# bilkitty/mj_envs

Hardware: AMD Instinct MI355X
Metric: env-steps/sec at N parallel envs, hammer-v0, 1/2/4/8 MI355X (higher is better)
Workload: dtype f32

## Files before the change

include/adroit_wave.h:

```cpp
#ifndef ADROIT_WAVE_H
#define ADROIT_WAVE_H

#include <stddef.h>
#include <stdint.h>

#ifdef __cplusplus
extern "C" {
#endif

typedef struct aw_handle aw_handle;

enum {
  AW_OK = 0,
  AW_EINVAL = -1,
  AW_EBLOB = -2,
  AW_EHIP = -3,
  AW_ENOMEM = -4,
  AW_EUNSUPPORTED = -5
};

enum {
  AW_ST_BADQPOS = 1,
  AW_ST_BADQVEL = 2,
  AW_ST_BADQACC = 4,
// ... 121 lines not shown
                         uint64_t seed, uint64_t draw, float* col, float* light, float* look, void* stream);

int aw_render_entries(const aw_handle* h, int* ngeom, int* nsite);
int aw_render_labels(aw_handle* h, const aw_view* views, int nviews, const float* env_cam,
                     const int32_t* env_ids, int n_sel, const int32_t* lut, int32_t background,
                     int sites, int width, int height, int32_t* labels, float* depth, void* stream);

#define AW_CLOUD_MAXCAND 8192
#define AW_FPS_MAXPOINTS 1024
int aw_render_cloud(aw_handle* h, const aw_view* views, int nviews, const float* env_cam,
                    const int32_t* env_ids, int n_sel, const uint8_t* keep, const float* box,
                    int frame_body, int sites, int width, int height, int cap, float* xyz, int32_t* pix,
                    int32_t* count, void* stream);
int aw_cloud_fps(int n, int cap, const float* xyz, const int32_t* count, int npoints, float* out_xyz,
                 int32_t* out_idx, void* stream);

#define AW_MAX_RAYS 256
typedef struct { float pnt[3], vec[3]; float xmax; int32_t body; uint64_t keep; } aw_ray_rec;
int aw_set_rays(aw_handle* h, const aw_ray_rec* rays, int nrays);
int aw_cast_rays(aw_handle* h, const int32_t* env_ids, int n_sel, const float* env_rays, float* dist,
                 int32_t* entry, void* stream);

int aw_policy_mlp(int n, int in_dim, int hidden, int out_dim, const float* params, const float* obs,
                  float* act, int sample, uint64_t seed, uint64_t step, uint64_t env_offset, void* stream);

#define AW_MAXPAIRCON 8
int aw_collide_test(aw_handle* h, int n, const int32_t* types, const float* pos, const float* mat,
                    const float* size, const float* margin, float* out, int32_t* count, double* out64,
                    void* stream);

int aw_midphase_test(aw_handle* h, int n, const int32_t* pair, const float* pos, const float* quat,
                     const float* size, int32_t* info, float* margin, void* stream);

int aw_stage_profile(unsigned long long* out, int reset);

const char* aw_last_error(void);

#ifdef __cplusplus
}
#endif

#endif
```

mj_envs_amd/_native.py:

```python
from __future__ import annotations

import ctypes
import os
from typing import Optional

import numpy as np

HERE = os.path.dirname(os.path.abspath(__file__))
LIB_PATH = os.environ.get("AW_LIB") or os.path.join(HERE, "libadroit_hip.so")

AW_NDIMS = 21
MAXCON, MAXEFC, MAXDENSE = 48, 192, 128
NCONMAX, NJMAX = 100, 500
ST_BADQPOS, ST_BADQVEL, ST_BADQACC, ST_CON_OVERFLOW, ST_EFC_OVERFLOW, ST_WIDE = 1, 2, 4, 8, 16, 32
ST_OVERFLOW = ST_CON_OVERFLOW | ST_EFC_OVERFLOW


def dump_layout(maxcon=MAXCON, maxefc=MAXEFC):
    c, e = 1768, 1768 + 14 * maxcon
    return dict(xpos=(0, 96), xquat=(96, 128), site_xpos=(224, 96), qacc_smooth=(320, 36),
                qfrc_smooth=(356, 36), qacc=(392, 36), qfrc_constraint=(428, 36), qM=(464, 1296),
                scalars=(1760, 8), con_dist=(c, maxcon), con_pos=(c + maxcon, 3 * maxcon),
                con_frame=(c + 4 * maxcon, 9 * maxcon), con_pair=(c + 13 * maxcon, maxcon),
                efc_force=(e, maxefc), efc_aref=(e + maxefc, maxefc), efc_D=(e + 2 * maxefc, maxefc),
# ... 86 lines not shown
    "aw_random_actions": (_i, [_vp, _u64, _u64, _vp, _vp]),
    "aw_set_env_offset": (_i, [_vp, _u64]),
    "aw_get_state": (_i, [_vp] * 6),
    "aw_set_state": (_i, [_vp] * 7),
    "aw_set_state_ids": (_i, [_vp, _vp, _i, _vp, _i, _vp, _vp, _vp, _vp, _i, _vp, _vp]),
    "aw_get_state_ids": (_i, [_vp, _vp, _i, _vp, _vp, _vp, _vp, _vp]),
    "aw_clone_envs": (_i, [_vp, _vp, _vp, _i, _i, _vp, _vp]),
    "aw_status": (_i, [_vp] * 4),
    "aw_clear_status": (_i, [_vp, _vp]),
    "aw_episode_stats": (_i, [_vp] * 6),
    "aw_episode_totals": (_i, [_vp] * 5),
    "aw_set_episode_totals": (_i, [_vp] * 5),
    "aw_get_episode": (_i, [_vp] * 6),
    "aw_set_episode": (_i, [_vp] * 6),
    "aw_task_eval": (_i, [_vp, _i] + [_vp] * 11),
    "aw_forward_dump": (_i, [_vp, _i, _vp, _vp, _vp]),
    "aw_forward_dump_wide": (_i, [_vp, _i, _vp, _vp, _vp]),
    "aw_dynamics": (_i, [_vp, _vp, _i, _P(DynPoint), _i, _vp, _vp, _vp, _P(DynOut), _vp]),
    "aw_render_depth": (_i, [_vp, _vp, _i, _i, _vp, _vp]),
    "aw_render_rgb": (_i, [_vp, _vp, _vp, _i, _i, _i, _vp, _vp, _vp]),
    "aw_render_views": (_i, [_vp, _P(View), _i, _vp, _vp, _i, _i, _i, _vp, _vp, _vp]),
    "aw_set_appearance": (_i, [_vp, _P(AppearanceBufs), _i]),
    "aw_appearance_defaults": (_i, [_vp, _vp, _vp, _P(_i)]),
    "aw_appearance_sample": (_i, [_vp, _vp, _vp, _vp, _i, _u64, _u64, _vp, _vp, _vp, _vp]),
    "aw_render_entries": (_i, [_vp, _P(_i), _P(_i)]),
    "aw_render_labels": (_i, [_vp, _P(View), _i, _vp, _vp, _i, _vp, _i, _i, _i, _i, _vp, _vp, _vp]),
    "aw_render_cloud": (_i, [_vp, _P(View), _i, _vp, _vp, _i, _vp, _vp] + [_i] * 5 + [_vp] * 4),
    "aw_cloud_fps": (_i, [_i, _i, _vp, _vp, _i, _vp, _vp, _vp]),
    "aw_set_rays": (_i, [_vp, _vp, _i]),
    "aw_cast_rays": (_i, [_vp, _vp, _i, _vp, _vp, _vp, _vp]),
    "aw_policy_mlp": (_i, [_i] * 4 + [_vp, _vp, _vp, _i, _u64, _u64, _u64, _vp]),
    "aw_collide_test": (_i, [_vp, _i] + [_vp] * 9),
    "aw_midphase_test": (_i, [_vp, _i] + [_vp] * 7),
    "aw_stage_profile": (_i, [_vp, _i]),
    "aw_last_error": (ctypes.c_char_p, []),
}
EXPORTS = tuple(ABI)


def data_groups(data) -> int:
    if data is None or data is False:
        return 0
    if data is True:
        return AW_DATA_ALL
    if isinstance(data, int):
        if data & ~AW_DATA_ALL or data < 0:
            raise ValueError(f"data: unknown group bits in {data}")
        return data
    names = (data,) if isinstance(data, str) else tuple(data)
    g = 0
    for k in names:
        if k not in DATA_GROUPS:
            raise ValueError(f"data: unknown group {k!r} (one of {sorted(DATA_GROUPS)})")
        g |= DATA_GROUPS[k]
    return g


class NativeError(RuntimeError):
    pass


def load():
    global _lib
    if _lib is not None:
        return _lib
    if not os.path.exists(LIB_PATH):
# ... 433 lines not shown
        _check(load().aw_render_cloud(self.h, arr, nv, _ptr(env_cam), _ptr(env_ids), n if n_sel is None else int(n_sel),
                                      _host_ptr(kp), _host_ptr(bx), int(frame_body), int(sites), w, h,
                                      0 if cap is None else int(cap), _ptr(xyz), _ptr(pix), _ptr(count), _stream()))

    def collide_test(self, types, pos, mat, size, margin, fp64: bool = False):
        import torch
        n = len(types)
        dev = self.torch_device
        t = lambda a, dt=torch.float32: torch.tensor(np.asarray(a), dtype=dt, device=dev).contiguous()
        out = torch.zeros(n, 8, 7, device=dev)
        cnt = torch.zeros(n, dtype=torch.int32, device=dev)
        out64 = torch.zeros(n, 8, 7, dtype=torch.float64, device=dev) if fp64 else None
        args = [t(types, torch.int32), t(pos), t(mat), t(size), t(margin)]
        _check(load().aw_collide_test(self.h, n, *[_ptr(a) for a in args], _ptr(out), _ptr(cnt), _ptr(out64),
                                      _stream()))
        o = (out64 if fp64 else out).cpu().numpy().astype(np.float64)
        c = cnt.cpu().numpy()
        return [o[i, :c[i]] for i in range(n)]

    def midphase_test(self, pair, pos, quat, size):
        import torch
        n = len(pair)
        dev = self.torch_device
        t = lambda a, dt=torch.float32: torch.tensor(np.asarray(a), dtype=dt, device=dev).contiguous()
        args = [t(pair, torch.int32), t(pos), t(quat), t(size)]
        _require(args[1].numel() == 6 * n and args[2].numel() == 8 * n and args[3].numel() == 6 * n,
                 "midphase_test: pos [n, 2, 3], quat [n, 2, 4], size [n, 2, 3]")
        info = torch.zeros(n, 6, dtype=torch.int32, device=dev)
        mg = torch.zeros(n, device=dev)
        _check(load().aw_midphase_test(self.h, n, *[_ptr(a) for a in args], _ptr(info), _ptr(mg), _stream()))
        i = info.cpu().numpy()
        return dict(keep=i[:, 0], g1=i[:, 1], g2=i[:, 2], cls=i[:, 3], type1=i[:, 4], type2=i[:, 5],
                    margin=mg.cpu().numpy())

    def dynamics(self, out: dict, points=(), env_ids=None, qpos=None, qvel=None, ctrl=None,
                 n_sel: Optional[int] = None, npoints: Optional[int] = None):
        import torch
        pts = list(points)
        arr = (DynPoint * max(len(pts), 1))()
        for k, (kind, idx) in enumerate(pts):
            arr[k].kind, arr[k].id = int(kind), int(idx)
        n, npt = self._n_sel("dynamics", env_ids), len(pts)
        unknown = set(out) - set(DYN_OUTPUTS)
        _require(not unknown, f"dynamics: unknown outputs {sorted(unknown)}")
        c = DynOut()
        for k, t in out.items():
            if _dev(t, f"dynamics: {k}", torch.float32, (n,) + dyn_shape(k, self.nv, self.nbody, npt)) is not None:
                setattr(c, k, t.data_ptr())
        self._rows("dynamics", n, qpos=qpos, qvel=qvel, ctrl=ctrl)
        _check(load().aw_dynamics(self.h, _ptr(env_ids), n if n_sel is None else int(n_sel), arr,
                                  npt if npoints is None else int(npoints), _ptr(qpos), _ptr(qvel), _ptr(ctrl),
                                  ctypes.byref(c), _stream()))

    def set_rays(self, records, nrays: Optional[int] = None):
        rec = None if records is None else np.ascontiguousarray(records, RAY_DTYPE).ravel()
        n = (0 if rec is None else int(rec.size)) if nrays is None else int(nrays)
        _require(rec is None or n <= rec.size or n > AW_MAX_RAYS, "set_rays: nrays exceeds the records given")
        _check(load().aw_set_rays(self.h, None if rec is None or rec.size == 0 else rec.ctypes.data, n))
        self.nrays = n

    def cast_rays(self, dist, entry=None, env_ids=None, env_rays=None, n_sel: Optional[int] = None):
        import torch
        n, R = self._n_sel("cast_rays", env_ids), getattr(self, "nrays", 0)
        _dev(dist, "cast_rays: dist", torch.float32, (n, R))
        _dev(entry, "cast_rays: entry", torch.int32, (n, R))
        _dev(env_rays, "cast_rays: env_rays", torch.float32, (self.n_envs, R, 6))
# ... 28 lines not shown
```

mj_envs_amd/csrc/aw_api.hip:

```cpp
#include <hip/hip_runtime.h>

#include <cmath>
#include <cstddef>
#include <cstdio>
#include <cstdlib>
#include <cstring>
#include <initializer_list>
#include <memory>
#include <string>
#include <vector>

#include "../../include/adroit_wave.h"
#include "../../include/aw_blob.h"
#include "aw_collide.h"
#include "aw_common.h"
#include "aw_handle.h"
#include "aw_model_host.h"
#include "aw_policy.h"
#include "aw_task.h"

using namespace aw;

__global__ void __launch_bounds__(64) k_task_eval(DModel m, int n, const float* qpos, const float* qvel,
                                                  const float* xpos, const float* xquat, const float* sxpos,
                                                  const float* touch, float* obs, float* reward, uint8_t* done,
                                                  uint8_t* goal) {
  __shared__ Env s;
  const int i = blockIdx.x, lane = threadIdx.x;
  if (i >= n) return;
  if (lane < m.nq) { s.qpos[lane] = qpos[(size_t)i * m.nq + lane]; s.qlo[lane] = 0.f; }
  if (lane < m.nv) s.qvel[lane] = qvel[(size_t)i * m.nv + lane];
  for (int k = lane; k < m.nbody * 3; k += 64) (&s.xpos[0][0])[k] = xpos[(size_t)i * m.nbody * 3 + k];
  for (int k = lane; k < m.nbody * 4; k += 64) (&s.xquat[0][0])[k] = xquat[(size_t)i * m.nbody * 4 + k];
  for (int k = lane; k < m.nsite * 3; k += 64) (&s.sxpos[0][0])[k] = sxpos[(size_t)i * m.nsite * 3 + k];
  if (lane == 0) s.touch[0] = touch ? touch[i] : 0.f;
  wsync();
  write_obs(m, s, lane, obs + (size_t)i * m.obs_dim);
  if (lane == 0) {
    float r;
    int dn, gl;
    task_reward(m, s, &r, &dn, &gl);
    reward[i] = r; done[i] = (uint8_t)dn; goal[i] = (uint8_t)gl;
  }
}

AW_DEV void collide_gv(const DModel& m, const GV& a, const GV& b, float margin, Emit& e, int gl) {
  const int lo = a.type, hi = b.type;
  if (hi == GEOM_BOX && lo == GEOM_CAPSULE) {
    c_capsule_box(a, b, margin, e, gl);
    return;
  }
  if (lo != GEOM_PLANE && (lo == GEOM_CYLINDER || hi == GEOM_CYLINDER)) {
// ... 46 lines not shown
  }
  wsync();
  const int nc = s.ncon < MAXPAIRCON ? s.ncon : MAXPAIRCON;
  if (lane == 0) count[i] = nc;
  if (lane < nc) {
    float* o = out + ((size_t)i * MAXPAIRCON + s.con_key[lane]) * 7;
    o[0] = s.con_dist[lane];
    for (int k = 0; k < 3; k++) { o[1 + k] = s.con_pos[lane][k]; o[4 + k] = s.con_nrm[lane][k]; }
  }
}

__global__ void __launch_bounds__(64) k_midphase_test(DModel m, int n, const int* pair, const float* pos,
                                                      const float* quat, const float* size, int* info,
                                                      float* margin) {
  __shared__ Env s;
  const int i = blockIdx.x, lane = threadIdx.x;
  if (i >= n || lane != 0) return;
  const int p = pair[i];
  if ((unsigned)p >= (unsigned)m.npairall) { info[6 * i] = -1; return; }
  const int g[2] = {MD(cp_g1, p), MD(cp_g2, p)};
  for (int q = 0; q < 2; q++) {
    for (int k = 0; k < 3; k++) { s.gxpos[g[q]][k] = pos[6 * i + 3 * q + k]; s.gsize[g[q]][k] = size[6 * i + 3 * q + k]; }
    for (int k = 0; k < 4; k++) s.gxquat[g[q]][k] = quat[8 * i + 4 * q + k];
  }
  const int cls = MD(cp_class, p);
  bool keep = true;
  if (cls == 2) keep = capbox_may_touch(m, s, p);
  else if (cls == 3) keep = boxbox_may_touch(m, s, p);
  else if (cls == 4) keep = mpr_may_touch(m, s, p);
  int* o = info + 6 * i;
  o[0] = keep ? 1 : 0; o[1] = g[0]; o[2] = g[1]; o[3] = cls;
  o[4] = MD(geom_type, g[0]); o[5] = MD(geom_type, g[1]);
  margin[i] = MD(cp_margin, p);
}

__global__ void k_random_actions(int n, int nu, uint64_t seed, uint64_t step, uint64_t env_offset, float* out) {
  int env = blockIdx.x * blockDim.x + threadIdx.x;
  if (env >= n) return;
  const uint32_t genv = (uint32_t)(env_offset + (uint64_t)env);
  for (int blk = 0; blk * 4 < nu; blk++) {
    uint32_t c[4] = {genv, (uint32_t)step, (uint32_t)(step >> 32), (uint32_t)blk};
    philox(c, (uint32_t)seed, (uint32_t)(seed >> 32));
    for (int k = 0; k < 4 && blk * 4 + k < nu; k++) out[(size_t)env * nu + blk * 4 + k] = 2.f * u01(c[k]) - 1.f;
  }
}

AW_DEV float appearance_draw(const float* lo, const float* hi, int i, uint32_t genv, uint64_t seed, uint64_t draw) {
  uint32_t c[4] = {genv, (uint32_t)draw, 0xA99Eu, (uint32_t)(i >> 2)};
  philox(c, (uint32_t)seed, (uint32_t)(seed >> 32));
  return lo[i] + (hi[i] - lo[i]) * u01(c[i & 3]);
}
__global__ void __launch_bounds__(256) k_appearance(int n, int nc, int nl, const float* __restrict__ lo,
                                                    const float* __restrict__ hi, const int* __restrict__ env_ids,
                                                    int row0, uint64_t env_offset, uint64_t seed, uint64_t draw, float* col,
                                                    float* light, float* look) {
  const int i = blockIdx.x * blockDim.x + threadIdx.x, F = nc + nl + AW_LOOK_FLOATS;
  const int row = row0 + (int)blockIdx.y;
  const int env = env_ids ? env_ids[row] : row;
  if (i >= F || (unsigned)env >= (unsigned)n) return;
  const uint32_t genv = (uint32_t)(env_offset + (uint64_t)env);
  float v = appearance_draw(lo, hi, i, genv, seed, draw);
  if (i < nc) {
    if (col) col[(size_t)env * nc + i] = v;
  } else if (i < nc + nl) {
    const int k = (i - nc) % LIGHT_W;
    if (k == 18 || k == 20 || k == 21) v = lo[i];
// ... 840 lines not shown
  const int bs = 256, nb = (n + bs - 1) / bs;
  hipStream_t st = (hipStream_t)stream;
  switch (hidden) {
    case 32: hipLaunchKernelGGL(k_mlp<32>, dim3(nb), dim3(bs), 0, st, n, in_dim, out_dim, params, obs, act, sample, seed, step, env_offset); break;
    case 64: hipLaunchKernelGGL(k_mlp<64>, dim3(nb), dim3(bs), 0, st, n, in_dim, out_dim, params, obs, act, sample, seed, step, env_offset); break;
    default: return fail(AW_EUNSUPPORTED, "aw_policy_mlp: hidden width must be 32 or 64 (two hidden layers)");
  }
  HIPCHK(hipGetLastError());
  return AW_OK;
}

int aw_collide_test(aw_handle* h, int n, const int32_t* types, const float* pos, const float* mat, const float* size,
                    const float* margin, float* out, int32_t* count, double* out64, void* stream) {
  if (!h || n <= 0 || !types || !pos || !mat || !size || !margin || !out || !count)
    return fail(AW_EINVAL, "aw_collide_test: bad arguments");
  HIPCHK(hipSetDevice(h->device));
  hipStream_t st = (hipStream_t)stream;
  hipLaunchKernelGGL(k_collide_test, dim3(n), dim3(64), 0, st, h->m, n, types, pos, mat, size, margin, out, count, out64);
  HIPCHK(hipGetLastError());
  return AW_OK;
}

int aw_midphase_test(aw_handle* h, int n, const int32_t* pair, const float* pos, const float* quat, const float* size,
                     int32_t* info, float* margin, void* stream) {
  if (!h || n <= 0 || !pair || !pos || !quat || !size || !info || !margin)
    return fail(AW_EINVAL, "aw_midphase_test: bad arguments");
  HIPCHK(hipSetDevice(h->device));
  hipStream_t st = (hipStream_t)stream;
  hipLaunchKernelGGL(k_midphase_test, dim3(n), dim3(64), 0, st, h->m, n, pair, pos, quat, size, info, margin);
  HIPCHK(hipGetLastError());
  return AW_OK;
}

int aw_stage_profile(unsigned long long* out, int reset) {
#ifdef AW_STAGE_PROF
  HIPCHK(stage_prof_read(out, reset));
  return AW_OK;
#else
  (void)out; (void)reset;
  return fail(AW_EUNSUPPORTED, "library built without -DAW_STAGE_PROF");
#endif
}

}
```

mj_envs_amd/csrc/aw_common.h:

```cpp
#pragma once
#include <hip/hip_runtime.h>
#include <stdint.h>

#define AW_DEV __device__ __attribute__((always_inline)) inline

namespace aw {

constexpr int MAXV = 36;
constexpr int CHOL_P = 4;
constexpr int VS = 36;
constexpr int MAXB = 32;
constexpr int MAXG = 36;
constexpr int MAXS = 32;
constexpr int MAXT = 44;
constexpr int MAXU = 30;
constexpr int MAXJB = 6;
constexpr int MAXP = 8;
constexpr int MAXLEV = 16;
constexpr int MAXTOUCH = 4;
constexpr int MAXSENS = 72;
constexpr int MAXPAIRCON = 8;
constexpr int NCLASS = 5;

}
// ... 197 lines not shown
                   \
  X(const SensTab*, sens, 1)                                                                      \
            \
  X(const DataTab*, data, 1)

typedef float MRec __attribute__((ext_vector_type(4)));

struct SensTab {
  int n;
  float* out;
  int type[MAXSENS], obj[MAXSENS], adr[MAXSENS];
  int site_type[MAXS];
  float site_size[MAXS * 3];
  int act_dof[MAXU];
};

struct DataTab {
  int groups, max_contacts;
  float *xpos, *xquat, *site_xpos, *qacc, *qfrc_constraint;
  int* counts;
  MRec* contact;
  int geom_id[MAXG];
};

struct MData {
#define AW_X(T, name, n) T name[n];
  AW_MODEL_ARRAYS(AW_X)
#undef AW_X
};

#ifndef AW_MD_AS
#define AW_MD_AS 4
#endif
template <class T>
AW_DEV T mld(const T* base, unsigned i) {
  typedef const __attribute__((address_space(AW_MD_AS))) T GT;
  typedef const __attribute__((address_space(AW_MD_AS))) char GC;
  return *(GT*)((GC*)base + i * (unsigned)sizeof(T));
}
#define MD(name, idx) ::aw::mld(m.d->name, (unsigned)(idx))
template <class T> using gp_t = __attribute__((address_space(1))) T*;
template <class T> AW_DEV gp_t<const T> gcp(const T* p) { return (gp_t<const T>)p; }
template <class T> AW_DEV gp_t<T> gmp(T* p) { return (gp_t<T>)p; }
#define MDP(name, idx) ::aw::gcp(&m.d->name[idx])
#define SENSTAB() ((const __attribute__((address_space(AW_MD_AS)))::aw::SensTab*)MD(sens, 0))
#define DATATAB() ((const __attribute__((address_space(AW_MD_AS)))::aw::DataTab*)MD(data, 0))
#ifndef AW_IO_GLOBAL
#define AW_IO_GLOBAL 1
#endif
#if AW_IO_GLOBAL
#define GIN(p) ::aw::gcp(p)
#define GOUT(p) ::aw::gmp(p)
#else
#define GIN(p) (p)
#define GOUT(p) (p)
#endif

struct DModel {
  int nq, nv, nu, nbody, njnt, ngeom, nsite, ntendon, npairall, nlevel;
  int nfl;
  int ntouch;
  int ndraw;
  int task_kind, frame_skip, horizon, obs_dim, nparam, variation;
  int success_steps;
  int iterations, noslip_iterations, mpr_iterations, disableflags;
  float timestep, gravity[3], tolerance, noslip_tolerance, mpr_tolerance, meaninertia;
  float pen_length, tar_length;
  double mpr_tolerance64;
  int cls_start[NCLASS + 1];
  int nrgeom;
// ... 300 lines not shown
```

mj_envs_amd/csrc/aw_solver.h:

```cpp
#pragma once
#include "aw_common.h"
#include "aw_dynamics.h"
#include "aw_tree.h"

namespace aw {

template <int NV>
AW_DEV void chol_factor(float (&row)[NV], int lane_in, float& invd, Env& s) {
  const int lane = opaque(lane_in);
  constexpr int P = CHOL_P;
  static_assert(sizeof(s.colbuf) >= (size_t)MAXV * P * 4, "panel buffer");
  float4* pan = s.colbuf;
#pragma unroll
  for (int j0 = 0; j0 < NV; j0 += P) {
    float a[P], u[P];
#pragma unroll
    for (int t = 0; t < P; t++) {
      const int j = j0 + t;
      a[t] = u[t] = 0.f;
      if (j < NV) {
        const float dj = __builtin_amdgcn_fmed3f(rlane(row[j], j), MINVAL, 3.402823466e38f);
        const float inv = __builtin_amdgcn_rcpf(dj);
        a[t] = row[j];
        if (lane == j) invd = inv;
// ... 761 lines not shown
  constexpr int NPL = 64 - NV;
  constexpr int XS = (NV + 3) & ~3;
  static_assert(NPL * XS * sizeof(float) <= offsetof(Env, qpos), "xd transpose buffer exceeds the phase-K/S union");
  float* Xb = reinterpret_cast<float*>(&s);
  const int nsparse = s.nsparse, ndense = s.ndense;
  float Am[NV];
  {
    float row[NV];
    float invd;
#if AW_MFAC_HANDOFF
    mfac_load<NV>(m, s, lane, row, invd);
#else
#pragma unroll
    for (int k = 0; k < NV; k++) row[k] = Mrow[k];
    tree_factor<TASK>(row, invd, lane);
#endif
    tree_inverse<TASK>(row, invd, lane, Am);
  }
  if (lane >= NV) {
#pragma unroll
    for (int k = 0; k < NV; k++) Am[k] = 0.f;
  }
  const int li = lane < NV ? lane : 0;
  const float lm = lane < NV ? 1.f : 0.f;
  wsync();
  AW_PROF(s, PR_NS_MINV);
  const bool use_fl = !(m.disableflags & DSBL_FRICTIONLOSS);
  const int flrow = lane < NV ? MD(fl_row, lane) : -1;
  const bool has_fl = flrow >= 0 && flrow < nsparse;
  float ca = 0.f, cb = 0.f, lim = 0.f, fa = 0.f, fb = 0.f, diag = 0.f;
  int rowe = 0;
  {
    float dg = 0.f;
#pragma unroll
    for (int k = 0; k < NV; k++) dg = k == lane ? Am[k] : dg;
    if (has_fl) { fa = s.efc_force[flrow]; fb = -fa; }
    if (use_fl && has_fl && dg >= MINVAL) {
      ca = 1.0f / dg;
      cb = s.efc_aref[flrow] * ca;
      lim = s.efc_floss[flrow];
      diag = dg;
    } else if (lane < NV) {
      lim = 3.0e38f;
    }
  }
  float R = lane < NV ? qacc : 0.f;
  auto jval = [&](int d) { return lm * (d < JL ? s.J[d][li] : jspill_row(m, s, d)[li]); };
  auto pair_col = [&](int e, float& jd, float& col) {
    float a = 0.f;
    if (e + 1 < JL) {
#pragma unroll
      for (int j = 0; j < NV; j++) a = fmaf(Am[j], s.J[e][j] - s.J[e + 1][j], a);
      jd = lm * (s.J[e][li] - s.J[e + 1][li]);
    } else {
      const float dl = jval(e) - jval(e + 1);
#pragma unroll
      for (int j = 0; j < NV; j++) a = fmaf(Am[j], rlane(dl, j), a);
      jd = dl;
    }
    col = a;
  };
  unsigned long long cmask[NDCH];
#pragma unroll
  for (int h = 0; h < NDCH; h++) {
    const int e = lane + 64 * h;
    bool c = e + 1 < ndense;
    if (c) c = s.efc_type[nsparse + e] == C_CON_PYRAMIDAL && s.efc_i1[nsparse + e] == 1;
    cmask[h] = __ballot(c);
  }
  int npr = 0;
  constexpr int NXCH = (MAXDENSE / 2 - NPL + 63) / 64 > 0 ? (MAXDENSE / 2 - NPL + 63) / 64 : 1;
  int ex_e[NXCH];
  float ex_ca[NXCH], ex_cb[NXCH], ex_K[NXCH], ex_fa[NXCH], ex_fb[NXCH];
#pragma unroll
  for (int xc = 0; xc < NXCH; xc++) { ex_e[xc] = 0; ex_ca[xc] = ex_cb[xc] = ex_K[xc] = ex_fa[xc] = ex_fb[xc] = 0.f; }
  int npr_all = 0;
#pragma unroll
  for (int h = 0; h < NDCH; h++) npr_all += __popcll(cmask[h]);
  constexpr bool X_FIT = NPL <= 32 && (NV > 32 ? NV : 32) * XS * sizeof(float) <= offsetof(Env, qpos);
  const bool x_mfma = X_FIT && (npr_all < NPL ? npr_all : NPL) >= 4;
#pragma unroll
  for (int h = 0; h < NDCH; h++) {
    unsigned long long mk = cmask[h];
    while (mk) {
      const int e = 64 * h + __builtin_ctzll(mk);
      mk &= mk - 1ull;
      const int p = npr++;
      if (p < NPL) {
        if (!x_mfma) {
          float jd, xd;
// ... 517 lines not shown
```

mj_envs_amd/csrc/aw_tree.h:

```cpp
#pragma once
#include <utility>

#include "aw_common.h"
#include "aw_trees.h"

namespace aw {

template <int TASK> struct Tree {
  using D = TreeDef<TASK>;
  static constexpr int NV = D::NV;
  static constexpr int depth(int j) {
    int d = 0;
    for (int p = D::parent[j]; p >= 0; p = D::parent[p]) d++;
    return d;
  }
  static constexpr int anc(int j, int a) {
    int p = D::parent[j];
    for (int t = 0; t < a; t++) p = D::parent[p];
    return p;
  }
  static constexpr int maxdepth() {
    int m = 0;
    for (int j = 0; j < NV; j++) m = depth(j) > m ? depth(j) : m;
    return m;
  }
  static constexpr int NLEV = maxdepth() + 1;
  static constexpr int split() {
    for (int p = 1; p < NV; p++) {
      bool ok = D::parent[p] < 0;
      for (int j = p; j < NV; j++)
        if (D::parent[j] >= 0 && D::parent[j] < p) ok = false;
      if (ok) return p;
    }
    return 0;
  }
  static constexpr int SPLIT = split();
  static constexpr bool ordered() {
    for (int j = 0; j < NV; j++)
      if (D::parent[j] >= j) return false;
    return true;
  }
};
template <int TASK, int J> struct TDepth { static constexpr int v = Tree<TASK>::depth(J); };
template <int TASK, int J, int A> struct TAnc { static constexpr int v = Tree<TASK>::anc(J, A); };

namespace tree {
template <int TASK> using Row = float[Tree<TASK>::NV];

template <int J> AW_DEV float below(float lf) { return __builtin_amdgcn_fmed3f((float)J - lf, 0.f, 1.f); }
template <int J> AW_DEV float above(float lf) { return __builtin_amdgcn_fmed3f(lf - (float)J, 0.f, 1.f); }
template <int J> AW_DEV float is(float lf) { return fmaxf(1.f - fabsf((float)J - lf), 0.f); }

template <int TASK, int J, int... A>
AW_DEV void col(Row<TASK>& r, float inv, float lf, std::integer_sequence<int, A...>) {
  const float c = r[J] * rlane(inv, J) * below<J>(lf);
  ((r[TAnc<TASK, J, A>::v] = fmaf(-c, rlane(r[TAnc<TASK, J, A>::v], J), r[TAnc<TASK, J, A>::v])), ...);
}
template <int TASK, int L, int J>
AW_DEV void col_at(Row<TASK>& r, float inv, float lf) {
  if constexpr (TDepth<TASK, J>::v == L && L > 0) col<TASK, J>(r, inv, lf, std::make_integer_sequence<int, L>{});
}
template <int TASK, int L, int J>
AW_DEV void piv_at(const Row<TASK>& r, float lf, float& d, float& e) {
  if constexpr (TDepth<TASK, J>::v == L) {
    const float f = is<J>(lf);
    d = fmaf(r[J], f, d);
    e += f;
  }
}
template <int TASK, int L, int... J>
AW_DEV void level(Row<TASK>& r, float& invd, float lf, std::integer_sequence<int, J...>) {
  float d = 0.f, e = 0.f;
  (piv_at<TASK, L, J>(r, lf, d, e), ...);
  const float inv = __builtin_amdgcn_rcpf(fmaxf(d, MINVAL));
  invd = fmaf(inv, e, invd);
  (col_at<TASK, L, J>(r, inv, lf), ...);
}
template <int TASK, int... Ls>
AW_DEV void levels_down(Row<TASK>& r, float& invd, float lf, std::integer_sequence<int, Ls...>) {
  constexpr int NL = Tree<TASK>::NLEV;
  (level<TASK, NL - 1 - Ls>(r, invd, lf, std::make_integer_sequence<int, Tree<TASK>::NV>{}), ...);
}

template <int TASK, int L, int J>
AW_DEV void up_at(const Row<TASK>& r, float invd, float& x, float lf) {
// ... 12 lines not shown
AW_DEV void down_at(const Row<TASK>& r, float invd, float& x, float lf) {
  if constexpr (TDepth<TASK, K>::v == L) x = fmaf(-r[K] * invd * above<K>(lf), rlane(x, K), x);
}
template <int TASK, int L, int... K>
AW_DEV void down_level(const Row<TASK>& r, float invd, float& x, float lf, std::integer_sequence<int, K...>) {
  (down_at<TASK, L, K>(r, invd, x, lf), ...);
}
template <int TASK, int... Ls>
AW_DEV void solve_down(const Row<TASK>& r, float invd, float& x, float lf, std::integer_sequence<int, Ls...>) {
  (down_level<TASK, Ls>(r, invd, x, lf, std::make_integer_sequence<int, Tree<TASK>::NV>{}), ...);
}

template <int TASK, int J, int... A>
AW_DEV void inv_up_col(const Row<TASK>& r, float invd, Row<TASK>& X, std::integer_sequence<int, A...>) {
  const float t = X[J] * rlane(invd, J);
  ((X[TAnc<TASK, J, A>::v] = fmaf(-rlane(r[TAnc<TASK, J, A>::v], J), t, X[TAnc<TASK, J, A>::v])), ...);
}
template <int TASK, int J, int... A>
AW_DEV void inv_down_col(const Row<TASK>& r, float invd, Row<TASK>& X, std::integer_sequence<int, A...>) {
  float acc = 0.f;
  ((acc = fmaf(rlane(r[TAnc<TASK, J, A>::v], J), X[TAnc<TASK, J, A>::v], acc)), ...);
  X[J] = fmaf(-rlane(invd, J), acc, X[J]);
}
template <int TASK, int... J>
AW_DEV void inverse_cols(const Row<TASK>& r, float invd, Row<TASK>& X, float lf, std::integer_sequence<int, J...>) {
  constexpr int NV = Tree<TASK>::NV;
  ((X[J] = is<J>(lf)), ...);
  ((inv_up_col<TASK, NV - 1 - J>(r, invd, X, std::make_integer_sequence<int, TDepth<TASK, NV - 1 - J>::v>{})), ...);
  ((X[J] *= rlane(invd, J)), ...);
  ((inv_down_col<TASK, J>(r, invd, X, std::make_integer_sequence<int, TDepth<TASK, J>::v>{})), ...);
}
}

template <int TASK>
AW_DEV void tree_factor(float (&r)[Tree<TASK>::NV], float& invd, int lane) {
  static_assert(Tree<TASK>::ordered(), "dof tree must list ancestors before descendants");
  invd = 0.f;
  tree::levels_down<TASK>(r, invd, opaque((float)lane), std::make_integer_sequence<int, Tree<TASK>::NLEV>{});
}
template <int TASK>
AW_DEV float tree_solve(const float (&r)[Tree<TASK>::NV], float invd, float b, int lane) {
  constexpr int NV = Tree<TASK>::NV, NL = Tree<TASK>::NLEV;
  const float lf = opaque((float)lane);
  float x = lane < NV ? b : 0.f;
  tree::solve_up<TASK>(r, invd, x, lf, std::make_integer_sequence<int, NL>{});
  x *= invd;
  tree::solve_down<TASK>(r, invd, x, lf, std::make_integer_sequence<int, NL>{});
  return lane < NV ? x : 0.f;
}
template <int TASK>
AW_DEV void tree_inverse(const float (&r)[Tree<TASK>::NV], float invd, int lane, float (&X)[Tree<TASK>::NV]) {
  tree::inverse_cols<TASK>(r, invd, X, opaque((float)lane), std::make_integer_sequence<int, Tree<TASK>::NV>{});
}

}
```

Baseline: 4.093 million.

## Batch cross-lane reads in tree factor/solve/inverse ahead of dependent FMAs

Adds a batched variant of the sparse tree LDL factor, solve and inverse that issues groups of up to eight cross-lane reads (rlane) at once. A scheduling barrier separates them from the FMAs that consume them, so permute latencies overlap instead of serializing per element. The solve now walks dofs grouped by tree level, and the solver's diagonal extraction and dot product use the same batching. It is enabled by default through AW_RL_BATCH. A tree_test kernel and API compare the serial and batched forms, and an optional SGPR base hint for model-data loads is added. The cost is more live registers per batch, which could lower occupancy.

```diff
diff --git a/include/adroit_wave.h b/include/adroit_wave.h
--- a/include/adroit_wave.h
+++ b/include/adroit_wave.h
@@ -177,6 +177,9 @@
 int aw_midphase_test(aw_handle* h, int n, const int32_t* pair, const float* pos, const float* quat,
                      const float* size, int32_t* info, float* margin, void* stream);
 
+#define AW_TREE_TEST_FLOATS(nv) (2 * (nv) * (nv) + 4 * (nv))
+int aw_tree_test(aw_handle* h, int n, const float* M, const float* b, const float* dd, float* out, void* stream);
+
 int aw_stage_profile(unsigned long long* out, int reset);
 
 const char* aw_last_error(void);
diff --git a/mj_envs_amd/_native.py b/mj_envs_amd/_native.py
--- a/mj_envs_amd/_native.py
+++ b/mj_envs_amd/_native.py
@@ -142,6 +142,7 @@
     "aw_policy_mlp": (_i, [_i] * 4 + [_vp, _vp, _vp, _i, _u64, _u64, _u64, _vp]),
     "aw_collide_test": (_i, [_vp, _i] + [_vp] * 9),
     "aw_midphase_test": (_i, [_vp, _i] + [_vp] * 7),
+    "aw_tree_test": (_i, [_vp, _i] + [_vp] * 5),
     "aw_stage_profile": (_i, [_vp, _i]),
     "aw_last_error": (ctypes.c_char_p, []),
 }
@@ -641,6 +642,26 @@
         i = info.cpu().numpy()
         return dict(keep=i[:, 0], g1=i[:, 1], g2=i[:, 2], cls=i[:, 3], type1=i[:, 4], type2=i[:, 5],
                     margin=mg.cpu().numpy())
+
+    def tree_test(self, M, b, dd):
+        import torch
+        nv = self.nv
+        dev = self.torch_device
+        t = lambda a: torch.tensor(np.asarray(a, np.float32), dtype=torch.float32, device=dev).contiguous()
+        args = [t(M), t(b), t(dd)]
+        n = args[1].shape[0]
+        _require(args[0].shape == (n, nv, nv) and args[1].shape == (n, nv) and args[2].shape == (n, nv),
+                 "tree_test: M [n, nv, nv], b [n, nv], dd [n, nv]")
+        w = 2 * nv * nv + 4 * nv
+        out = torch.zeros(n, 2, w, device=dev)
+        _check(load().aw_tree_test(self.h, n, *[_ptr(a) for a in args], _ptr(out), _stream()))
+        o = out.cpu().numpy()
+        res = []
+        for f in range(2):
+            v = o[:, f, 2 * nv * nv:].reshape(n, 4, nv)
+            res.append(dict(factor=o[:, f, :nv * nv].reshape(n, nv, nv), inverse=o[:, f, nv * nv:2 * nv * nv].reshape(n, nv, nv),
+                            invd=v[:, 0], x=v[:, 1], invd_damped=v[:, 2], x_damped=v[:, 3]))
+        return res
 
     def dynamics(self, out: dict, points=(), env_ids=None, qpos=None, qvel=None, ctrl=None,
                  n_sel: Optional[int] = None, npoints: Optional[int] = None):
diff --git a/mj_envs_amd/csrc/aw_api.hip b/mj_envs_amd/csrc/aw_api.hip
--- a/mj_envs_amd/csrc/aw_api.hip
+++ b/mj_envs_amd/csrc/aw_api.hip
@@ -18,6 +18,7 @@
 #include "aw_model_host.h"
 #include "aw_policy.h"
 #include "aw_task.h"
+#include "aw_tree.h"
 
 using namespace aw;
 
@@ -130,6 +131,38 @@
   o[0] = keep ? 1 : 0; o[1] = g[0]; o[2] = g[1]; o[3] = cls;
   o[4] = MD(geom_type, g[0]); o[5] = MD(geom_type, g[1]);
   margin[i] = MD(cp_margin, p);
+}
+
+template <int TASK, bool SERIAL>
+AW_DEV void tree_test_form(const float (&Mrow)[Tree<TASK>::NV], float b, float dd, int lane, float* o) {
+  constexpr int NV = Tree<TASK>::NV;
+  float row[NV], rd[NV], X[NV], invd, invd2;
+#pragma unroll
+  for (int k = 0; k < NV; k++) { row[k] = Mrow[k]; rd[k] = Mrow[k] + (k == lane ? dd : 0.f); }
+  tree_factor<TASK, SERIAL>(row, invd, lane);
+  const float x = tree_solve<TASK, SERIAL>(row, invd, b, lane);
+  tree_inverse<TASK, SERIAL>(row, invd, lane, X);
+  tree_factor<TASK, SERIAL>(rd, invd2, lane);
+  const float x2 = tree_solve<TASK, SERIAL>(rd, invd2, b, lane);
+  if (lane < NV) {
+#pragma unroll
+    for (int k = 0; k < NV; k++) { o[lane * NV + k] = row[k]; o[(NV + lane) * NV + k] = X[k]; }
+    float* v = o + 2 * NV * NV;
+    v[lane] = invd; v[NV + lane] = x; v[2 * NV + lane] = invd2; v[3 * NV + lane] = x2;
+  }
+}
+template <int TASK>
+__global__ void __launch_bounds__(64) k_tree_test(int n, const float* M, const float* b, const float* dd, float* out) {
+  constexpr int NV = Tree<TASK>::NV, W = AW_TREE_TEST_FLOATS(NV);
+  const int i = blockIdx.x, lane = threadIdx.x;
+  if (i >= n) return;
+  const int li = lane < NV ? lane : NV - 1;
+  float Mrow[NV];
+#pragma unroll
+  for (int k = 0; k < NV; k++) Mrow[k] = M[((size_t)i * NV + li) * NV + k];
+  const float bl = b[(size_t)i * NV + li], dl = dd[(size_t)i * NV + li];
+  tree_test_form<TASK, true>(Mrow, bl, dl, lane, out + ((size_t)i * 2 + 0) * W);
+  tree_test_form<TASK, false>(Mrow, bl, dl, lane, out + ((size_t)i * 2 + 1) * W);
 }
 
 __global__ void k_random_actions(int n, int nu, uint64_t seed, uint64_t step, uint64_t env_offset, float* out) {
@@ -1036,6 +1069,21 @@
   return AW_OK;
 }
 
+int aw_tree_test(aw_handle* h, int n, const float* M, const float* b, const float* dd, float* out, void* stream) {
+  if (!h || n <= 0 || !M || !b || !dd || !out) return fail(AW_EINVAL, "aw_tree_test: bad arguments");
+  HIPCHK(hipSetDevice(h->device));
+  hipStream_t st = (hipStream_t)stream;
+  switch (h->m.task_kind) {
+    case 0: hipLaunchKernelGGL(k_tree_test<0>, dim3(n), dim3(64), 0, st, n, M, b, dd, out); break;
+    case 1: hipLaunchKernelGGL(k_tree_test<1>, dim3(n), dim3(64), 0, st, n, M, b, dd, out); break;
+    case 2: hipLaunchKernelGGL(k_tree_test<2>, dim3(n), dim3(64), 0, st, n, M, b, dd, out); break;
+    case 3: hipLaunchKernelGGL(k_tree_test<3>, dim3(n), dim3(64), 0, st, n, M, b, dd, out); break;
+    default: return fail(AW_EINVAL, "aw_tree_test: unknown task");
+  }
+  HIPCHK(hipGetLastError());
+  return AW_OK;
+}
+
 int aw_stage_profile(unsigned long long* out, int reset) {
 #ifdef AW_STAGE_PROF
   HIPCHK(stage_prof_read(out, reset));
diff --git a/mj_envs_amd/csrc/aw_common.h b/mj_envs_amd/csrc/aw_common.h
--- a/mj_envs_amd/csrc/aw_common.h
+++ b/mj_envs_amd/csrc/aw_common.h
@@ -253,10 +253,18 @@
 #ifndef AW_MD_AS
 #define AW_MD_AS 4
 #endif
+#ifndef AW_SBASE
+#define AW_SBASE 0
+#endif
 template <class T>
 AW_DEV T mld(const T* base, unsigned i) {
   typedef const __attribute__((address_space(AW_MD_AS))) T GT;
   typedef const __attribute__((address_space(AW_MD_AS))) char GC;
+#if AW_SBASE == 2
+  asm volatile("" : "+s"(base));
+#elif AW_SBASE
+  asm("" : "+s"(base));
+#endif
   return *(GT*)((GC*)base + i * (unsigned)sizeof(T));
 }
 #define MD(name, idx) ::aw::mld(m.d->name, (unsigned)(idx))
diff --git a/mj_envs_amd/csrc/aw_solver.h b/mj_envs_amd/csrc/aw_solver.h
--- a/mj_envs_amd/csrc/aw_solver.h
+++ b/mj_envs_amd/csrc/aw_solver.h
@@ -817,8 +817,13 @@
   int rowe = 0;
   {
     float dg = 0.f;
+#if AW_RL_BATCH
+    const float lf = opaque((float)lane);
+    tree_diag<TASK>(Am, lf, dg, std::make_integer_sequence<int, NV>{});
+#else
 #pragma unroll
     for (int k = 0; k < NV; k++) dg = k == lane ? Am[k] : dg;
+#endif
     if (has_fl) { fa = s.efc_force[flrow]; fb = -fa; }
     if (use_fl && has_fl && dg >= MINVAL) {
       ca = 1.0f / dg;
@@ -839,8 +844,12 @@
       jd = lm * (s.J[e][li] - s.J[e + 1][li]);
     } else {
       const float dl = jval(e) - jval(e + 1);
+#if AW_RL_BATCH
+      a = tree::batch::dot_lanes<NV, 0>(Am, dl, a, tree::batch::Seq<tree::batch::take(NV, 0)>{});
+#else
 #pragma unroll
       for (int j = 0; j < NV; j++) a = fmaf(Am[j], rlane(dl, j), a);
+#endif
       jd = dl;
     }
     col = a;
diff --git a/mj_envs_amd/csrc/aw_tree.h b/mj_envs_amd/csrc/aw_tree.h
--- a/mj_envs_amd/csrc/aw_tree.h
+++ b/mj_envs_amd/csrc/aw_tree.h
@@ -25,6 +25,16 @@
     return m;
   }
   static constexpr int NLEV = maxdepth() + 1;
+  static constexpr int lev_count(int l) {
+    int n = 0;
+    for (int j = 0; j < NV; j++) n += depth(j) == l;
+    return n;
+  }
+  static constexpr int lev_dof(int l, int n) {
+    for (int j = 0; j < NV; j++)
+      if (depth(j) == l && n-- == 0) return j;
+    return -1;
+  }
   static constexpr int split() {
     for (int p = 1; p < NV; p++) {
       bool ok = D::parent[p] < 0;
@@ -43,6 +53,12 @@
 };
 template <int TASK, int J> struct TDepth { static constexpr int v = Tree<TASK>::depth(J); };
 template <int TASK, int J, int A> struct TAnc { static constexpr int v = Tree<TASK>::anc(J, A); };
+template <int TASK, int L> struct TLevCount { static constexpr int v = Tree<TASK>::lev_count(L); };
+template <int TASK, int L, int N> struct TLevDof { static constexpr int v = Tree<TASK>::lev_dof(L, N); };
+
+#ifndef AW_RL_BATCH
+#define AW_RL_BATCH 1
+#endif
 
 namespace tree {
 template <int TASK> using Row = float[Tree<TASK>::NV];
@@ -51,6 +67,7 @@
 template <int J> AW_DEV float above(float lf) { return __builtin_amdgcn_fmed3f(lf - (float)J, 0.f, 1.f); }
 template <int J> AW_DEV float is(float lf) { return fmaxf(1.f - fabsf((float)J - lf), 0.f); }
 
+namespace serial {
 template <int TASK, int J, int... A>
 AW_DEV void col(Row<TASK>& r, float inv, float lf, std::integer_sequence<int, A...>) {
   const float c = r[J] * rlane(inv, J) * below<J>(lf);
@@ -129,25 +146,162 @@
 }
 }
 
-template <int TASK>
+namespace batch {
+constexpr int RLB = 8;
+constexpr int take(int n, int a0) { return n - a0 < RLB ? n - a0 : RLB; }
+template <int N> using Seq = std::make_integer_sequence<int, N>;
+
+template <int TASK, int J, int A0, int... B>
+AW_DEV void col_part(Row<TASK>& r, float inv, float lf, float& c, std::integer_sequence<int, B...>) {
+  constexpr int N = TDepth<TASK, J>::v;
+  float ij = 0.f;
+  if constexpr (A0 == 0) ij = rlane(inv, J);
+  const float mj[] = {rlane(r[TAnc<TASK, J, A0 + B>::v], J)...};
+  __builtin_amdgcn_sched_barrier(0);
+  if constexpr (A0 == 0) c = r[J] * ij * below<J>(lf);
+  ((r[TAnc<TASK, J, A0 + B>::v] = fmaf(-c, mj[B], r[TAnc<TASK, J, A0 + B>::v])), ...);
+  if constexpr (A0 + RLB < N) col_part<TASK, J, A0 + RLB>(r, inv, lf, c, Seq<take(N, A0 + RLB)>{});
+}
+template <int TASK, int L, int J>
+AW_DEV void col_at(Row<TASK>& r, float inv, float lf) {
+  if constexpr (TDepth<TASK, J>::v == L && L > 0) {
+    float c;
+    col_part<TASK, J, 0>(r, inv, lf, c, Seq<take(L, 0)>{});
+  }
+}
+template <int TASK, int L, int... J>
+AW_DEV void level(Row<TASK>& r, float& invd, float lf, std::integer_sequence<int, J...>) {
+  float d = 0.f, e = 0.f;
+  (serial::piv_at<TASK, L, J>(r, lf, d, e), ...);
+  const float inv = __builtin_amdgcn_rcpf(fmaxf(d, MINVAL));
+  invd = fmaf(inv, e, invd);
+  (col_at<TASK, L, J>(r, inv, lf), ...);
+}
+template <int TASK, int... Ls>
+AW_DEV void levels_down(Row<TASK>& r, float& invd, float lf, std::integer_sequence<int, Ls...>) {
+  constexpr int NL = Tree<TASK>::NLEV;
+  (level<TASK, NL - 1 - Ls>(r, invd, lf, Seq<Tree<TASK>::NV>{}), ...);
+}
+
+template <int TASK, int L, int N0, int... B>
+AW_DEV void up_part(const Row<TASK>& r, float xs, float& x, float lf, std::integer_sequence<int, B...>) {
+  constexpr int N = TLevCount<TASK, L>::v;
+  const float xj[] = {rlane(xs, TLevDof<TASK, L, N0 + B>::v)...};
+  __builtin_amdgcn_sched_barrier(0);
+  ((x = fmaf(-r[TLevDof<TASK, L, N0 + B>::v] * below<TLevDof<TASK, L, N0 + B>::v>(lf), xj[B], x)), ...);
+  if constexpr (N0 + RLB < N) up_part<TASK, L, N0 + RLB>(r, xs, x, lf, Seq<take(N, N0 + RLB)>{});
+}
+template <int TASK, int... Ls>
+AW_DEV void solve_up(const Row<TASK>& r, float invd, float& x, float lf, std::integer_sequence<int, Ls...>) {
+  constexpr int NL = Tree<TASK>::NLEV;
+  ((up_part<TASK, NL - 1 - Ls, 0>(r, x * invd, x, lf, Seq<take(TLevCount<TASK, NL - 1 - Ls>::v, 0)>{})), ...);
+}
+template <int TASK, int L, int N0, int... B>
+AW_DEV void down_part(const Row<TASK>& r, float invd, float& x, float lf, std::integer_sequence<int, B...>) {
+  constexpr int N = TLevCount<TASK, L>::v;
+  const float xk[] = {rlane(x, TLevDof<TASK, L, N0 + B>::v)...};
+  __builtin_amdgcn_sched_barrier(0);
+  ((x = fmaf(-r[TLevDof<TASK, L, N0 + B>::v] * invd * above<TLevDof<TASK, L, N0 + B>::v>(lf), xk[B], x)), ...);
+  if constexpr (N0 + RLB < N) down_part<TASK, L, N0 + RLB>(r, invd, x, lf, Seq<take(N, N0 + RLB)>{});
+}
+template <int TASK, int... Ls>
+AW_DEV void solve_down(const Row<TASK>& r, float invd, float& x, float lf, std::integer_sequence<int, Ls...>) {
+  ((down_part<TASK, Ls, 0>(r, invd, x, lf, Seq<take(TLevCount<TASK, Ls>::v, 0)>{})), ...);
+}
+
+template <int TASK, int J, int A0, int... B>
+AW_DEV void inv_up_part(const Row<TASK>& r, float invd, Row<TASK>& X, float& t, std::integer_sequence<int, B...>) {
+  constexpr int N = TDepth<TASK, J>::v;
+  float ij = 0.f;
+  if constexpr (A0 == 0) ij = rlane(invd, J);
+  const float mj[] = {rlane(r[TAnc<TASK, J, A0 + B>::v], J)...};
+  __builtin_amdgcn_sched_barrier(0);
+  if constexpr (A0 == 0) t = X[J] * ij;
+  ((X[TAnc<TASK, J, A0 + B>::v] = fmaf(-mj[B], t, X[TAnc<TASK, J, A0 + B>::v])), ...);
+  if constexpr (A0 + RLB < N) inv_up_part<TASK, J, A0 + RLB>(r, invd, X, t, Seq<take(N, A0 + RLB)>{});
+}
+template <int TASK, int J>
+AW_DEV void inv_up_col(const Row<TASK>& r, float invd, Row<TASK>& X) {
+  if constexpr (TDepth<TASK, J>::v > 0) {
+    float t;
+    inv_up_part<TASK, J, 0>(r, invd, X, t, Seq<take(TDepth<TASK, J>::v, 0)>{});
+  }
+}
+template <int TASK, int J, int A0, int... B>
+AW_DEV void inv_down_part(const Row<TASK>& r, float invd, Row<TASK>& X, float& acc, std::integer_sequence<int, B...>) {
+  constexpr int N = TDepth<TASK, J>::v;
+  const float mj[] = {rlane(r[TAnc<TASK, J, A0 + B>::v], J)...};
+  float ij = 0.f;
+  if constexpr (A0 + RLB >= N) ij = rlane(invd, J);
+  __builtin_amdgcn_sched_barrier(0);
+  ((acc = fmaf(mj[B], X[TAnc<TASK, J, A0 + B>::v], acc)), ...);
+  if constexpr (A0 + RLB < N) inv_down_part<TASK, J, A0 + RLB>(r, invd, X, acc, Seq<take(N, A0 + RLB)>{});
+  else X[J] = fmaf(-ij, acc, X[J]);
+}
+template <int TASK, int J>
+AW_DEV void inv_down_col(const Row<TASK>& r, float invd, Row<TASK>& X) {
+  float acc = 0.f;
+  if constexpr (TDepth<TASK, J>::v == 0) X[J] = fmaf(-rlane(invd, J), acc, X[J]);
+  else inv_down_part<TASK, J, 0>(r, invd, X, acc, Seq<take(TDepth<TASK, J>::v, 0)>{});
+}
+template <int TASK, int J0, int... B>
+AW_DEV void inv_scale_part(float invd, Row<TASK>& X, std::integer_sequence<int, B...>) {
+  constexpr int NV = Tree<TASK>::NV;
+  const float ij[] = {rlane(invd, J0 + B)...};
+  __builtin_amdgcn_sched_barrier(0);
+  ((X[J0 + B] *= ij[B]), ...);
+  if constexpr (J0 + RLB < NV) inv_scale_part<TASK, J0 + RLB>(invd, X, Seq<take(NV, J0 + RLB)>{});
+}
+template <int TASK, int... J>
+AW_DEV void inverse_cols(const Row<TASK>& r, float invd, Row<TASK>& X, float lf, std::integer_sequence<int, J...>) {
+  constexpr int NV = Tree<TASK>::NV;
+  ((X[J] = is<J>(lf)), ...);
+  ((inv_up_col<TASK, NV - 1 - J>(r, invd, X)), ...);
+  inv_scale_part<TASK, 0>(invd, X, Seq<take(NV, 0)>{});
+  ((inv_down_col<TASK, J>(r, invd, X)), ...);
+}
+template <int NV, int J0, int... B>
+AW_DEV float dot_lanes(const float (&a)[NV], float x, float acc, std::integer_sequence<int, B...>) {
+  const float xj[] = {rlane(x, J0 + B)...};
+  __builtin_amdgcn_sched_barrier(0);
+  ((acc = fmaf(a[J0 + B], xj[B], acc)), ...);
+  if constexpr (J0 + RLB < NV) return dot_lanes<NV, J0 + RLB>(a, x, acc, Seq<take(NV, J0 + RLB)>{});
+  else return acc;
+}
+}
+}
+
+template <int TASK, int... J>
+AW_DEV void tree_diag(const float (&X)[Tree<TASK>::NV], float lf, float& d, std::integer_sequence<int, J...>) {
+  ((d = fmaf(X[J], tree::is<J>(lf), d)), ...);
+}
+
+template <int TASK, bool SERIAL = !AW_RL_BATCH>
 AW_DEV void tree_factor(float (&r)[Tree<TASK>::NV], float& invd, int lane) {
   static_assert(Tree<TASK>::ordered(), "dof tree must list ancestors before descendants");
   invd = 0.f;
-  tree::levels_down<TASK>(r, invd, opaque((float)lane), std::make_integer_sequence<int, Tree<TASK>::NLEV>{});
-}
-template <int TASK>
+  constexpr std::make_integer_sequence<int, Tree<TASK>::NLEV> levels{};
+  if constexpr (SERIAL) tree::serial::levels_down<TASK>(r, invd, opaque((float)lane), levels);
+  else tree::batch::levels_down<TASK>(r, invd, opaque((float)lane), levels);
+}
+template <int TASK, bool SERIAL = !AW_RL_BATCH>
 AW_DEV float tree_solve(const float (&r)[Tree<TASK>::NV], float invd, float b, int lane) {
-  constexpr int NV = Tree<TASK>::NV, NL = Tree<TASK>::NLEV;
+  constexpr int NV = Tree<TASK>::NV;
+  constexpr std::make_integer_sequence<int, Tree<TASK>::NLEV> levels{};
   const float lf = opaque((float)lane);
   float x = lane < NV ? b : 0.f;
-  tree::solve_up<TASK>(r, invd, x, lf, std::make_integer_sequence<int, NL>{});
+  if constexpr (SERIAL) tree::serial::solve_up<TASK>(r, invd, x, lf, levels);
+  else tree::batch::solve_up<TASK>(r, invd, x, lf, levels);
   x *= invd;
-  tree::solve_down<TASK>(r, invd, x, lf, std::make_integer_sequence<int, NL>{});
+  if constexpr (SERIAL) tree::serial::solve_down<TASK>(r, invd, x, lf, levels);
+  else tree::batch::solve_down<TASK>(r, invd, x, lf, levels);
   return lane < NV ? x : 0.f;
 }
-template <int TASK>
+template <int TASK, bool SERIAL = !AW_RL_BATCH>
 AW_DEV void tree_inverse(const float (&r)[Tree<TASK>::NV], float invd, int lane, float (&X)[Tree<TASK>::NV]) {
-  tree::inverse_cols<TASK>(r, invd, X, opaque((float)lane), std::make_integer_sequence<int, Tree<TASK>::NV>{});
-}
-
-}
+  constexpr std::make_integer_sequence<int, Tree<TASK>::NV> dofs{};
+  if constexpr (SERIAL) tree::serial::inverse_cols<TASK>(r, invd, X, opaque((float)lane), dofs);
+  else tree::batch::inverse_cols<TASK>(r, invd, X, opaque((float)lane), dofs);
+}
+
+}
```

Result: no change. 4.119 million (median of 6 runs) (+0.6%).
